# AcherStyx/SSD-Object-Detection

Measured on AMD Instinct MI355X. Metric: images/sec SSD300 train step, batch 64, higher is better.
Workload: dtype bf16; 1 GPU; BASELINE configs[2]: SSD300 full train step (anchor match+encode, image normalisation, conv fwd, loss, conv bwd, per-variable clip (64 variables) + Adam), per-GPU batch 64, 80 classes, synthetic COCO-shaped boxes; per_gpu_batch=64, global_batch=64, parallelism=single

## Files before the change

include/ssd_hip.h:

```cpp
#ifndef SSD_HIP_H
#define SSD_HIP_H

#include <stddef.h>
#include <stdint.h>

#ifdef __cplusplus
extern "C" {
#endif

typedef enum {
    SSD_OK = 0,
    SSD_ERR_ASSERT = -1,
    SSD_ERR_VALUE = -2,
    SSD_ERR_WORKSPACE = -3,
    SSD_ERR_LAUNCH = -4,
    SSD_ERR_UNSUPPORTED = -5
} ssd_status;

typedef enum { SSD_F32 = 0, SSD_BF16 = 1 } ssd_dtype;

int ssd_hip_abi_version(void);
const char* ssd_status_string(int status);

int ssd_priors_count(const int* grid_hw, int levels, const int* ratio_off);
// ... 88 lines not shown
    const void* x;
    const void* dy;
    float* dw;
    float* dbias;
    int B, H, W, Cin, Cout, ldy, ksize, stride, pad_t, pad_l, Ho, Wo;
} ssd_wgrad_item;
size_t ssd_conv2d_bwd_weight_batched_workspace_bytes(const ssd_wgrad_item* items, int count);
int ssd_conv2d_bwd_weight_batched(const ssd_wgrad_item* items, int count, void* ws, size_t ws_bytes, void* stream);
int ssd_set_wgrad_reduce_stream(void* stream);
int ssd_weight_transpose(const void* w, void* w_t, int Cout, int ksize, int Cin, int Cout_pad, void* stream);
int ssd_weight_transpose_batched(const long long* desc, int ntensors, int max_tiles, void* stream);
int ssd_cast_bf16(const float* src, void* dst, long long n, void* stream);
int ssd_image_prep(const float* img, void* out, int B, int H, int W, int normalize, void* stream);
int ssd_image_resize_prep(const void* src, const int64_t* src_off, const int32_t* src_hw, void* out, int B, int S,
                          int normalize, void* stream);
int ssd_box_prep(const float* box_tlwh, const int32_t* gt_off, const int32_t* src_hw, float* box_out, int B, int total_gt,
                 void* stream);
int ssd_maxpool2x2_fwd(const void* x, void* y, int B, int H, int W, int C, int Ho, int Wo, void* stream);
int ssd_maxpool2x2_bwd(const void* x, const void* y, const void* dy, void* dx, int B, int H, int W, int C, int Ho,
                       int Wo, void* stream);
int ssd_maxpool2x2_fwd_argmax(const void* x, void* y, void* code, int B, int H, int W, int C, int Ho, int Wo, void* stream);
int ssd_maxpool2x2_bwd_argmax(const void* code, const void* dy, void* dx, int B, int H, int W, int C, int Ho, int Wo,
                              void* stream);
int ssd_quantize_mx_fp8(const void* x_bf16, void* q, void* scale, long long n, void* stream);
int ssd_conv3x3_fwd_mxfp8(const void* x8, const void* xscale, const void* w8, const void* wscale, const float* bias, void* y, int B,
                          int H, int W, int Cin, int Cout, int relu, void* stream);
#define SSD_CHAIN_MAX_LAYERS 8
#define SSD_CHAIN_PACK_MAX 16
typedef struct {
    const void* src;
    void* dst;
    int N, K;
} ssd_chain_pack;
int ssd_chain_pack_weights(const ssd_chain_pack* items, int count, void* stream);
int ssd_chain_prefetch(const ssd_chain_pack* items, int count, void* stream);
typedef struct {
    const void* w;
    const float* bias;
    void* out;
    const void* mask_bits;
    const void* mask_src;
    void* relu_bits;
    int Hi, Wi, Kc, Ho, Wo, N, ksize, mul, div, pad_t, pad_l, relu, accumulate;
} ssd_chain_layer;
int ssd_conv_chain(const void* in0, const ssd_chain_layer* layers, int nlayers, int B, void* stream);
int ssd_add_relu_fwd(const void* a, const void* b, void* out, long long n, void* stream);
int ssd_relu_mask_bwd(const void* g, const void* act, void* out, int accumulate, long long n, void* stream);
int ssd_maxpool3x3s2_fwd(const void* x, void* y, void* code, int B, int H, int W, int C, int Ho, int Wo, int pad_t, int pad_l,
                         void* stream);
int ssd_maxpool3x3s2_bwd(const void* code, const void* dy, void* dx, int B, int H, int W, int C, int Ho, int Wo, int pad_t, int pad_l,
                         void* stream);
typedef struct {
    int levels;
    int H[SSD_MAX_LEVELS], W[SSD_MAX_LEVELS], Cin[SSD_MAX_LEVELS], cout[SSD_MAX_LEVELS];
    const void* x[SSD_MAX_LEVELS];
    const void* w_tap[SSD_MAX_LEVELS];
    const void* relu_bits[SSD_MAX_LEVELS];
    const void* relu_src[SSD_MAX_LEVELS];
    void* dx[SSD_MAX_LEVELS];
    float* dw[SSD_MAX_LEVELS];
    float* dbias[SSD_MAX_LEVELS];
} ssd_head_layers;
size_t ssd_heads_bwd_data_sparse_workspace_bytes(int B, const ssd_head_layers* hl);
int ssd_heads_bwd_data_sparse(const ssd_head_grads* hg, const ssd_head_layers* hl, int B, void* ws, size_t ws_bytes,
                              void* stream);
int ssd_heads_bwd_data_sparse_levels(const ssd_head_grads* hg, const ssd_head_layers* hl, int B, unsigned level_mask, int prezeroed,
                                     void* ws, size_t ws_bytes, void* stream);
size_t ssd_heads_bwd_weight_sparse_workspace_bytes(int B, const ssd_head_grads* hg, const ssd_head_layers* hl);
int ssd_heads_bwd_weight_sparse(const ssd_head_grads* hg, const ssd_head_layers* hl, int B, void* ws, size_t ws_bytes,
                                void* stream);

int ssd_head_grad_pack(const void* dloc, const void* dconf, void* out, int B, int hw, int per_cell, int classes,
                       int npad, int anchors_total, int level_off, void* stream);

int ssd_opt_block_elems(void);
int ssd_grad_clip_scales(const float* grad, long long n, const int32_t* tensor_block_off, int ntensors, float clip,
                         double* partial, float* scale, float* norms, void* stream);
int ssd_grad_apply_scale(float* grad, long long n, const int32_t* block_tensor, const float* scale, void* stream);
int ssd_grad_accumulate(float* acc, const float* grad, long long n, const int32_t* block_tensor, const float* scale,
                        int first, void* stream);
int ssd_adam_step(float* param, const float* grad, float* m, float* v, void* param_bf16, long long n,
                  const int32_t* block_tensor, const float* scale, float grad_scale, float lr_t, float beta1,
                  float beta2, float eps, void* stream);
int ssd_sgd_step(float* param, const float* grad, void* param_bf16, long long n, const int32_t* block_tensor,
                 const float* scale, float grad_scale, float lr, void* stream);

enum ssd_conv_plan {
    SSD_PLAN_KERNEL_MASK = 0xff,
    SSD_PLAN_C64B = 1, SSD_PLAN_P32_64, SSD_PLAN_P32_128, SSD_PLAN_8PH,
    SSD_PLAN_DMA_256_256, SSD_PLAN_DMA_256_128, SSD_PLAN_DMA_256_64, SSD_PLAN_DMA_128_64, SSD_PLAN_DMA_128_128,
    SSD_PLAN_CONV0_FWD, SSD_PLAN_P512, SSD_PLAN_PW,
    SSD_PLAN_WG_FIRST = 32, SSD_PLAN_WG_PATCH_16x16, SSD_PLAN_WG_PATCH_6x40, SSD_PLAN_WG_PATCH_10x24, SSD_PLAN_WG_TILE,
    SSD_PLAN_WG_GENERIC,
    SSD_PLAN_F_FLAT = 0x100,
    SSD_PLAN_F_ROWFLAT = 0x200,
    SSD_PLAN_F_SPLITK = 0x400,
    SSD_PLAN_F_POOL_FUSED = 0x800,
    SSD_PLAN_F_S2 = 0x1000,
    SSD_PLAN_F_REDUCE_WIDE = 0x2000
};
int ssd_conv2d_fwd_plan(int B, int H, int W, int Cin, int Cout, int ksize, int stride, int pad_t, int pad_l, int Ho, int Wo,
                        int pool, size_t ws_bytes);
int ssd_conv2d_head_fwd_plan(int B, int H, int W, int Cin, int per_cell, int classes, size_t ws_bytes);
int ssd_conv2d_bwd_data_plan(int B, int H, int W, int Cin, int Cout_pad, int ksize, int stride, int pad_t, int pad_l, int Ho,
                             int Wo, int accumulate, size_t ws_bytes);
int ssd_conv2d_bwd_weight_plan(int B, int H, int W, int Cin, int Cout, int ldy, int ksize, int stride, int pad_t, int pad_l,
                               int Ho, int Wo);
const char* ssd_conv_plan_name(int plan);

int ssd_dev_knob(const char* name, int value);

int ssd_dev_mfma_calibration_workgroups(void);
double ssd_dev_mfma_calibration_flops(int iters);
int ssd_dev_mfma_calibration(int iters, void* stamps, void* sink, void* stream);

#ifdef __cplusplus
}
#endif
#endif
```

ssd-object-detection_amd/_lib.py:

```python
import ctypes
import os

HERE = os.path.dirname(os.path.abspath(__file__))
LIB_PATH = os.path.join(HERE, os.environ.get("SSD_HIP_LIB", "libssd_hip.so"))

SSD_OK, SSD_ERR_ASSERT, SSD_ERR_VALUE, SSD_ERR_WORKSPACE, SSD_ERR_LAUNCH, SSD_ERR_UNSUPPORTED = 0, -1, -2, -3, -4, -5
SSD_MAX_LEVELS = 8

_c_int_p = ctypes.POINTER(ctypes.c_int)
_c_double_p = ctypes.POINTER(ctypes.c_double)
VP = ctypes.c_void_p


class PriorGrid(ctypes.Structure):
    _fields_ = [("levels", ctypes.c_int),
                ("grid_h", ctypes.c_int * SSD_MAX_LEVELS),
                ("grid_w", ctypes.c_int * SSD_MAX_LEVELS),
                ("per_cell", ctypes.c_int * SSD_MAX_LEVELS),
                ("verified", ctypes.c_int)]


class HeadGrads(ctypes.Structure):
    _fields_ = [("levels", ctypes.c_int),
                ("hw", ctypes.c_int * SSD_MAX_LEVELS),
# ... 17 lines not shown
                ("relu_src", VP * SSD_MAX_LEVELS),
                ("dx", VP * SSD_MAX_LEVELS),
                ("dw", VP * SSD_MAX_LEVELS),
                ("dbias", VP * SSD_MAX_LEVELS)]


class ChainLayer(ctypes.Structure):
    _fields_ = [("w", VP), ("bias", VP), ("out", VP), ("mask_bits", VP), ("mask_src", VP), ("relu_bits", VP)] + \
               [(n, ctypes.c_int) for n in ("Hi", "Wi", "Kc", "Ho", "Wo", "N", "ksize", "mul", "div", "pad_t", "pad_l", "relu",
                                            "accumulate")]


class WgradItem(ctypes.Structure):
    _fields_ = [("x", VP), ("dy", VP), ("dw", VP), ("dbias", VP)] + \
               [(n, ctypes.c_int) for n in ("B", "H", "W", "Cin", "Cout", "ldy", "ksize", "stride", "pad_t", "pad_l", "Ho", "Wo")]


class ChainPack(ctypes.Structure):
    _fields_ = [("src", VP), ("dst", VP), ("N", ctypes.c_int), ("K", ctypes.c_int)]


SSD_CHAIN_MAX_LAYERS = 8
SSD_CHAIN_PACK_MAX = 16
_HG = ctypes.POINTER(HeadGrads)
_HL = ctypes.POINTER(HeadLayers)

_SIGNATURES = {
    "ssd_hip_abi_version": (ctypes.c_int, []),
    "ssd_status_string": (ctypes.c_char_p, [ctypes.c_int]),
    "ssd_priors_count": (ctypes.c_int, [_c_int_p, ctypes.c_int, _c_int_p]),
    "ssd_priors": (ctypes.c_int, [_c_int_p, ctypes.c_int, _c_double_p, _c_int_p, _c_int_p, ctypes.c_double, VP, VP]),
    "ssd_encode_zero": (ctypes.c_int, [VP, ctypes.c_int, VP, VP]),
    "ssd_prior_grid_verify": (ctypes.c_int, [VP, ctypes.c_int, ctypes.POINTER(PriorGrid), VP, VP]),
    "ssd_match_encode_workspace_bytes": (ctypes.c_size_t, [ctypes.c_int, ctypes.c_int, ctypes.c_int]),
    "ssd_match_encode": (ctypes.c_int, [VP, VP, VP, ctypes.c_int, ctypes.c_int, ctypes.c_int, VP, VP, ctypes.c_int,
                                        ctypes.POINTER(PriorGrid), ctypes.c_double, VP, VP, VP, VP, VP, ctypes.c_size_t, VP]),
    "ssd_apply_anchor_box": (ctypes.c_int, [VP, VP, ctypes.c_int, VP, VP]),
    "ssd_iou_n": (ctypes.c_int, [VP, VP, ctypes.c_int, VP, VP]),
    "ssd_score_decode": (ctypes.c_int, [VP, VP, ctypes.c_int, VP, ctypes.c_int, ctypes.c_int, ctypes.c_int,
                                        ctypes.c_float, ctypes.c_double, VP, VP, VP, VP, VP]),
    "ssd_nms_max_candidates": (ctypes.c_int, []),
    "ssd_nms": (ctypes.c_int, [VP, VP, VP, VP, ctypes.c_int, ctypes.c_int, ctypes.c_float, ctypes.c_int, VP, VP, VP]),
    "ssd_conv2d_fwd": (ctypes.c_int, [VP, VP, VP, VP] + [ctypes.c_int] * 12 + [VP, ctypes.c_size_t, VP]),
    "ssd_conv2d_fwd_pool": (ctypes.c_int, [VP, VP, VP, VP, VP, VP] + [ctypes.c_int] * 14 + [VP, ctypes.c_size_t, VP]),
    "ssd_conv2d_head_fwd": (ctypes.c_int, [VP, VP, VP, VP, VP] + [ctypes.c_int] * 8 + [VP, ctypes.c_size_t, VP]),
    "ssd_conv2d_bwd_data": (ctypes.c_int, [VP, VP, VP, VP] + [ctypes.c_int] * 12 + [VP, ctypes.c_size_t, VP]),
    "ssd_conv2d_fwd_relubits": (ctypes.c_int, [VP] * 5 + [ctypes.c_int] * 11 + [VP, ctypes.c_size_t, VP]),
    "ssd_conv2d_bwd_data_bits": (ctypes.c_int, [VP] * 4 + [ctypes.c_int] * 12 + [VP, ctypes.c_size_t, VP]),
    "ssd_conv2d_bwd_data_unpool": (ctypes.c_int, [VP] * 6 + [ctypes.c_int] * 7 + [VP, ctypes.c_size_t, VP]),
    "ssd_quantize_mx_fp8": (ctypes.c_int, [VP, VP, VP, ctypes.c_longlong, VP]),
    "ssd_conv3x3_fwd_mxfp8": (ctypes.c_int, [VP] * 6 + [ctypes.c_int] * 6 + [VP]),
    "ssd_chain_pack_weights": (ctypes.c_int, [ctypes.POINTER(ChainPack), ctypes.c_int, VP]),
    "ssd_chain_prefetch": (ctypes.c_int, [ctypes.POINTER(ChainPack), ctypes.c_int, VP]),
    "ssd_set_wgrad_reduce_stream": (ctypes.c_int, [VP]),
    "ssd_conv2d_bwd_weight_batched_workspace_bytes": (ctypes.c_size_t, [ctypes.POINTER(WgradItem), ctypes.c_int]),
    "ssd_conv2d_bwd_weight_batched": (ctypes.c_int, [ctypes.POINTER(WgradItem), ctypes.c_int, VP, ctypes.c_size_t, VP]),
    "ssd_conv_chain": (ctypes.c_int, [VP, ctypes.POINTER(ChainLayer), ctypes.c_int, ctypes.c_int, VP]),
    "ssd_add_relu_fwd": (ctypes.c_int, [VP, VP, VP, ctypes.c_longlong, VP]),
    "ssd_relu_mask_bwd": (ctypes.c_int, [VP, VP, VP, ctypes.c_int, ctypes.c_longlong, VP]),
    "ssd_maxpool3x3s2_fwd": (ctypes.c_int, [VP, VP, VP] + [ctypes.c_int] * 8 + [VP]),
    "ssd_maxpool3x3s2_bwd": (ctypes.c_int, [VP, VP, VP] + [ctypes.c_int] * 8 + [VP]),
    "ssd_conv2d_bwd_weight_unpooled_workspace_bytes": (ctypes.c_size_t, [ctypes.c_int] * 7),
    "ssd_conv2d_bwd_weight_unpooled": (ctypes.c_int, [VP] * 5 + [ctypes.c_int] * 7 + [VP, ctypes.c_size_t, VP]),
    "ssd_conv2d_bwd_data_wgrad_first_workspace_bytes": (ctypes.c_size_t, [ctypes.c_int] * 3),
    "ssd_conv2d_bwd_data_wgrad_first": (ctypes.c_int, [VP] * 6 + [ctypes.c_int] * 3 + [VP, ctypes.c_size_t, VP]),
    "ssd_conv2d_bwd_weight_workspace_bytes": (ctypes.c_size_t, [ctypes.c_int] * 7),
    "ssd_conv2d_bwd_weight": (ctypes.c_int, [VP, VP, VP, VP] + [ctypes.c_int] * 12 + [VP, ctypes.c_size_t, VP]),
    "ssd_weight_transpose": (ctypes.c_int, [VP, VP, ctypes.c_int, ctypes.c_int, ctypes.c_int, ctypes.c_int, VP]),
    "ssd_cast_bf16": (ctypes.c_int, [VP, VP, ctypes.c_longlong, VP]),
    "ssd_image_prep": (ctypes.c_int, [VP, VP, ctypes.c_int, ctypes.c_int, ctypes.c_int, ctypes.c_int, VP]),
    "ssd_image_resize_prep": (ctypes.c_int, [VP, VP, VP, VP, ctypes.c_int, ctypes.c_int, ctypes.c_int, VP]),
    "ssd_box_prep": (ctypes.c_int, [VP, VP, VP, VP, ctypes.c_int, ctypes.c_int, VP]),
    "ssd_maxpool2x2_fwd": (ctypes.c_int, [VP, VP] + [ctypes.c_int] * 6 + [VP]),
    "ssd_maxpool2x2_bwd": (ctypes.c_int, [VP, VP, VP, VP] + [ctypes.c_int] * 6 + [VP]),
    "ssd_weight_transpose_batched": (ctypes.c_int, [VP, ctypes.c_int, ctypes.c_int, VP]),
    "ssd_maxpool2x2_fwd_argmax": (ctypes.c_int, [VP, VP, VP] + [ctypes.c_int] * 6 + [VP]),
    "ssd_maxpool2x2_bwd_argmax": (ctypes.c_int, [VP, VP, VP] + [ctypes.c_int] * 6 + [VP]),
    "ssd_head_grad_pack": (ctypes.c_int, [VP, VP, VP] + [ctypes.c_int] * 7 + [VP]),
    "ssd_opt_block_elems": (ctypes.c_int, []),
    "ssd_grad_clip_scales": (ctypes.c_int, [VP, ctypes.c_longlong, VP, ctypes.c_int, ctypes.c_float, VP, VP, VP, VP]),
    "ssd_grad_apply_scale": (ctypes.c_int, [VP, ctypes.c_longlong, VP, VP, VP]),
    "ssd_grad_accumulate": (ctypes.c_int, [VP, VP, ctypes.c_longlong, VP, VP, ctypes.c_int, VP]),
    "ssd_adam_step": (ctypes.c_int, [VP, VP, VP, VP, VP, ctypes.c_longlong, VP, VP] + [ctypes.c_float] * 5 + [VP]),
    "ssd_sgd_step": (ctypes.c_int, [VP, VP, VP, ctypes.c_longlong, VP, VP, ctypes.c_float, ctypes.c_float, VP]),
    "ssd_dev_knob": (ctypes.c_int, [ctypes.c_char_p, ctypes.c_int]),
    "ssd_dev_mfma_calibration_workgroups": (ctypes.c_int, []),
    "ssd_dev_mfma_calibration_flops": (ctypes.c_double, [ctypes.c_int]),
    "ssd_dev_mfma_calibration": (ctypes.c_int, [ctypes.c_int, VP, VP, VP]),
    "ssd_conv2d_fwd_plan": (ctypes.c_int, [ctypes.c_int] * 12 + [ctypes.c_size_t]),
    "ssd_conv2d_head_fwd_plan": (ctypes.c_int, [ctypes.c_int] * 6 + [ctypes.c_size_t]),
    "ssd_conv2d_bwd_data_plan": (ctypes.c_int, [ctypes.c_int] * 12 + [ctypes.c_size_t]),
    "ssd_conv2d_bwd_weight_plan": (ctypes.c_int, [ctypes.c_int] * 12),
    "ssd_conv_plan_name": (ctypes.c_char_p, [ctypes.c_int]),
    "ssd_loss_workspace_bytes": (ctypes.c_size_t, [ctypes.c_int, ctypes.c_int, ctypes.c_int]),
    "ssd_loss_heads_workspace_bytes": (ctypes.c_size_t, [ctypes.c_int, ctypes.c_int, ctypes.c_int]),
    "ssd_loss_fwd_bwd_heads": (ctypes.c_int, [VP, VP, ctypes.c_int, VP, VP, VP, ctypes.c_int, ctypes.c_int, ctypes.c_int,
                                              ctypes.c_float, VP, _HG, VP, ctypes.c_size_t, ctypes.c_int, VP]),
    "ssd_heads_bwd_data_sparse_workspace_bytes": (ctypes.c_size_t, [ctypes.c_int, _HL]),
    "ssd_heads_bwd_data_sparse": (ctypes.c_int, [_HG, _HL, ctypes.c_int, VP, ctypes.c_size_t, VP]),
    "ssd_heads_bwd_data_sparse_levels": (ctypes.c_int, [_HG, _HL, ctypes.c_int, ctypes.c_uint, ctypes.c_int, VP, ctypes.c_size_t, VP]),
    "ssd_heads_bwd_weight_sparse_workspace_bytes": (ctypes.c_size_t, [ctypes.c_int, _HG, _HL]),
    "ssd_heads_bwd_weight_sparse": (ctypes.c_int, [_HG, _HL, ctypes.c_int, VP, ctypes.c_size_t, VP]),
    "ssd_loss_fwd_bwd": (ctypes.c_int, [VP, VP, ctypes.c_int, VP, VP, VP, ctypes.c_int, ctypes.c_int, ctypes.c_int,
                                        ctypes.c_float, VP, VP, VP, VP, ctypes.c_size_t, VP]),
}

_lib = None


def lib():
    global _lib
    if _lib is None:
        if not os.path.exists(LIB_PATH):
            raise RuntimeError(
                "libssd_hip.so is missing (%s): build it with `python ssd-object-detection_amd/build.py` "
                "or __graft_entry__.build(); there is no CPU fallback." % LIB_PATH)
        try:
            import torch
        except ImportError:
            pass
        L = ctypes.CDLL(LIB_PATH)
        for name, (res, args) in _SIGNATURES.items():
            fn = getattr(L, name)
            fn.restype = res
            fn.argtypes = args
        _lib = L
    return _lib


def check(status):
    if status == SSD_OK:
        return
    msg = lib().ssd_status_string(status).decode()
    if status == SSD_ERR_ASSERT:
        raise AssertionError(msg)
    if status in (SSD_ERR_VALUE, SSD_ERR_UNSUPPORTED):
        raise ValueError(msg)
    raise RuntimeError("ssd_hip: %s (status %d)" % (msg, status))
```

ssd-object-detection_amd/csrc/optim.hip:

```cpp
#include "common.h"
#include <hip/hip_bf16.h>

namespace {

constexpr int OPT_BLOCK = 1024;

__device__ __forceinline__ unsigned short f2bf_bits(float f) {
    const __hip_bfloat16 h = __float2bfloat16(f);
    return *reinterpret_cast<const unsigned short*>(&h);
}

__global__ __launch_bounds__(256) void k_sqnorm_partial(const float* __restrict__ g, long long n, double* __restrict__ partial) {
    __shared__ double s_red[4];
    const long long i = ((long long)blockIdx.x * 256 + threadIdx.x) * 4;
    double s = 0.0;
    if (i + 3 < n) {
        const float4 v = *reinterpret_cast<const float4*>(g + i);
        s = (double)v.x * v.x + (double)v.y * v.y + (double)v.z * v.z + (double)v.w * v.w;
    } else {
        for (long long k = i; k < n; ++k) s += (double)g[k] * g[k];
    }
#pragma unroll
    for (int off = 32; off > 0; off >>= 1) {
        const int lo = __shfl_xor(__double2loint(s), off);
        const int hi = __shfl_xor(__double2hiint(s), off);
        s += __hiloint2double(hi, lo);
    }
    if ((threadIdx.x & 63) == 0) s_red[threadIdx.x >> 6] = s;
    __syncthreads();
    if (threadIdx.x == 0) partial[blockIdx.x] = s_red[0] + s_red[1] + s_red[2] + s_red[3];
}

__global__ __launch_bounds__(256) void k_clip_scale(const double* __restrict__ partial, const int* __restrict__ tensor_block_off,
                                                    int ntensors, float clip, float* __restrict__ scale,
                                                    float* __restrict__ norms) {
    __shared__ double s_red[256];
    const int t = blockIdx.x;
    if (t >= ntensors) return;
    const int b0 = tensor_block_off[t], b1 = tensor_block_off[t + 1];
    double s = 0.0;
    for (int b = b0 + threadIdx.x; b < b1; b += 256) s += partial[b];
    s_red[threadIdx.x] = s;
    __syncthreads();
    for (int off = 128; off > 0; off >>= 1) {
        if (threadIdx.x < off) s_red[threadIdx.x] += s_red[threadIdx.x + off];
        __syncthreads();
    }
    if (threadIdx.x == 0) {
        const float nrm = (float)sqrt(s_red[0]);
        if (norms) norms[t] = nrm;
        scale[t] = clip > 0.f ? clip / fmaxf(nrm, clip) : 1.f;
    }
}

__global__ __launch_bounds__(256) void k_apply_scale(float* __restrict__ g, long long n, const int* __restrict__ block_tensor,
                                                     const float* __restrict__ scale) {
    const long long i = ((long long)blockIdx.x * 256 + threadIdx.x) * 4;
    if (i >= n) return;
    const float sc = scale[block_tensor[blockIdx.x]];
    float4 v = *reinterpret_cast<float4*>(g + i);
    v.x *= sc; v.y *= sc; v.z *= sc; v.w *= sc;
    *reinterpret_cast<float4*>(g + i) = v;
}

__global__ __launch_bounds__(256) void k_accumulate(float* __restrict__ acc, const float* __restrict__ g, long long n,
                                                    const int* __restrict__ block_tensor, const float* __restrict__ scale,
                                                    int first) {
    const long long i = ((long long)blockIdx.x * 256 + threadIdx.x) * 4;
    if (i >= n) return;
    const float sc = scale ? scale[block_tensor[blockIdx.x]] : 1.f;
    const float4 gv = *reinterpret_cast<const float4*>(g + i);
    float4 a = first ? make_float4(0.f, 0.f, 0.f, 0.f) : *reinterpret_cast<float4*>(acc + i);
    a.x += gv.x * sc; a.y += gv.y * sc; a.z += gv.z * sc; a.w += gv.w * sc;
    *reinterpret_cast<float4*>(acc + i) = a;
}

__global__ __launch_bounds__(256) void k_adam(float* __restrict__ p, const float* __restrict__ g, float* __restrict__ m,
                                              float* __restrict__ v, unsigned short* __restrict__ p_bf16, long long n,
                                              const int* __restrict__ block_tensor, const float* __restrict__ scale,
                                              float grad_scale, float lr_t, float b1, float b2, float eps) {
    const long long i = ((long long)blockIdx.x * 256 + threadIdx.x) * 4;
    if (i >= n) return;
    const float sc = grad_scale * (scale ? scale[block_tensor[blockIdx.x]] : 1.f);
    const float4 gv = *reinterpret_cast<const float4*>(g + i);
    float4 pv = *reinterpret_cast<float4*>(p + i);
    float4 mv = *reinterpret_cast<float4*>(m + i);
    float4 vv = *reinterpret_cast<float4*>(v + i);
    const float gs[4] = {gv.x * sc, gv.y * sc, gv.z * sc, gv.w * sc};
    float* pp = reinterpret_cast<float*>(&pv);
    float* mm = reinterpret_cast<float*>(&mv);
    float* vq = reinterpret_cast<float*>(&vv);
#pragma unroll
    for (int k = 0; k < 4; ++k) {
        mm[k] = b1 * mm[k] + (1.f - b1) * gs[k];
        vq[k] = b2 * vq[k] + (1.f - b2) * gs[k] * gs[k];
        pp[k] -= lr_t * mm[k] / (sqrtf(vq[k]) + eps);
    }
    *reinterpret_cast<float4*>(p + i) = pv;
    *reinterpret_cast<float4*>(m + i) = mv;
    *reinterpret_cast<float4*>(v + i) = vv;
    if (p_bf16)
        *reinterpret_cast<uint2*>(p_bf16 + i) = make_uint2((unsigned)f2bf_bits(pp[0]) | ((unsigned)f2bf_bits(pp[1]) << 16),
                                                           (unsigned)f2bf_bits(pp[2]) | ((unsigned)f2bf_bits(pp[3]) << 16));
}

__global__ __launch_bounds__(256) void k_sgd(float* __restrict__ p, const float* __restrict__ g, unsigned short* __restrict__ p_bf16,
                                             long long n, const int* __restrict__ block_tensor, const float* __restrict__ scale,
                                             float grad_scale, float lr) {
    const long long i = ((long long)blockIdx.x * 256 + threadIdx.x) * 4;
    if (i >= n) return;
    const float sc = grad_scale * (scale ? scale[block_tensor[blockIdx.x]] : 1.f);
    const float4 gv = *reinterpret_cast<const float4*>(g + i);
    float4 pv = *reinterpret_cast<float4*>(p + i);
    pv.x -= lr * gv.x * sc; pv.y -= lr * gv.y * sc; pv.z -= lr * gv.z * sc; pv.w -= lr * gv.w * sc;
    *reinterpret_cast<float4*>(p + i) = pv;
    if (p_bf16)
        *reinterpret_cast<uint2*>(p_bf16 + i) = make_uint2((unsigned)f2bf_bits(pv.x) | ((unsigned)f2bf_bits(pv.y) << 16),
                                                           (unsigned)f2bf_bits(pv.z) | ((unsigned)f2bf_bits(pv.w) << 16));
}

}

extern "C" {

int ssd_opt_block_elems(void) { return OPT_BLOCK; }

int ssd_grad_clip_scales(const float* grad, long long n, const int32_t* tensor_block_off, int ntensors, float clip,
                         double* partial, float* scale, float* norms, void* stream) {
    if (!grad || !tensor_block_off || !partial || !scale || n <= 0 || n % OPT_BLOCK || ntensors <= 0) return SSD_ERR_VALUE;
    const unsigned nb = (unsigned)(n / OPT_BLOCK);
    hipStream_t s = (hipStream_t)stream;
    hipLaunchKernelGGL(k_sqnorm_partial, dim3(nb), dim3(256), 0, s, grad, n, partial);
    hipLaunchKernelGGL(k_clip_scale, dim3(ntensors), dim3(256), 0, s, partial, tensor_block_off, ntensors, clip,
                       scale, norms);
    return ssd_launch_status();
}

int ssd_grad_apply_scale(float* grad, long long n, const int32_t* block_tensor, const float* scale, void* stream) {
    if (!grad || !block_tensor || !scale || n <= 0 || n % OPT_BLOCK) return SSD_ERR_VALUE;
    hipLaunchKernelGGL(k_apply_scale, dim3((unsigned)(n / OPT_BLOCK)), dim3(256), 0, (hipStream_t)stream, grad, n,
                       block_tensor, scale);
    return ssd_launch_status();
}

int ssd_grad_accumulate(float* acc, const float* grad, long long n, const int32_t* block_tensor, const float* scale,
                        int first, void* stream) {
    if (!acc || !grad || n <= 0 || n % OPT_BLOCK || (scale && !block_tensor)) return SSD_ERR_VALUE;
    hipLaunchKernelGGL(k_accumulate, dim3((unsigned)(n / OPT_BLOCK)), dim3(256), 0, (hipStream_t)stream, acc, grad, n,
                       block_tensor, scale, first);
    return ssd_launch_status();
}

int ssd_adam_step(float* param, const float* grad, float* m, float* v, void* param_bf16, long long n,
                  const int32_t* block_tensor, const float* scale, float grad_scale, float lr_t, float beta1, float beta2,
                  float eps, void* stream) {
    if (!param || !grad || !m || !v || n <= 0 || n % OPT_BLOCK || (scale && !block_tensor)) return SSD_ERR_VALUE;
    hipLaunchKernelGGL(k_adam, dim3((unsigned)(n / OPT_BLOCK)), dim3(256), 0, (hipStream_t)stream, param, grad, m, v,
                       static_cast<unsigned short*>(param_bf16), n, block_tensor, scale, grad_scale, lr_t, beta1, beta2, eps);
    return ssd_launch_status();
}

int ssd_sgd_step(float* param, const float* grad, void* param_bf16, long long n, const int32_t* block_tensor,
                 const float* scale, float grad_scale, float lr, void* stream) {
    if (!param || !grad || n <= 0 || n % OPT_BLOCK || (scale && !block_tensor)) return SSD_ERR_VALUE;
    hipLaunchKernelGGL(k_sgd, dim3((unsigned)(n / OPT_BLOCK)), dim3(256), 0, (hipStream_t)stream, param, grad,
                       static_cast<unsigned short*>(param_bf16), n, block_tensor, scale, grad_scale, lr);
    return ssd_launch_status();
}

}
```

ssd-object-detection_amd/engine.py:

```python
import ctypes
import math
import os

import numpy as np
import torch

from . import _lib, ops

SSD300_TRUNK = [
    ("conv", 8, 64, 3, 1, "same", False),
    ("conv", 64, 64, 3, 1, "same", False),
    ("pool", 64, 64, 2, 2, "valid", False),
    ("conv", 64, 128, 3, 1, "same", False),
    ("conv", 128, 128, 3, 1, "same", False),
    ("pool", 128, 128, 2, 2, "valid", False),
    ("conv", 128, 256, 3, 1, "same", False),
    ("conv", 256, 256, 3, 1, "same", False),
    ("conv", 256, 256, 3, 1, "same", False),
    ("pool", 256, 256, 2, 2, "same", False),
    ("conv", 256, 512, 3, 1, "same", False),
    ("conv", 512, 512, 3, 1, "same", False),
    ("conv", 512, 512, 1, 1, "same", True),
    ("conv", 512, 1024, 3, 2, "same", False),
    ("conv", 1024, 1024, 1, 1, "same", True),
# ... 138 lines not shown
        for i, nd in enumerate(self.nodes):
            if nd["kind"] != "conv":
                continue
            self.conv_params[i] = (add("conv%d/kernel" % i, (nd["cout"], nd["k"], nd["k"], nd["cin"])),
                                   add("conv%d/bias" % i, (nd["cout"],)))
        self.head_params = []
        for lvl, ((_, h, c), n) in enumerate(zip(self.fm, self.num_priors)):
            nl, nc = n * 4, n * self.classes
            lk, ck = add("head%d/loc_kernel" % lvl, (nl, 3, 3, c), True), add("head%d/conf_kernel" % lvl, (nc, 3, 3, c))
            lb, cb = add("head%d/loc_bias" % lvl, (nl,), True), add("head%d/conf_bias" % lvl, (nc,))
            self.head_params.append((FusedView("head%d/kernel" % lvl, (nl + nc, 3, 3, c), (lk, ck)),
                                     FusedView("head%d/bias" % lvl, (nl + nc,), (lb, cb))))
        self.n_flat = off
        self.n_params = sum(t.numel for t in self.tensors)

    def _alloc_params(self):
        dev, n = self.device, self.n_flat
        self.param = torch.zeros(n, dtype=torch.float32, device=dev)
        self.grad = torch.zeros(n, dtype=torch.float32, device=dev)
        self.grad_acc = None
        self.adam_m = torch.zeros(n, dtype=torch.float32, device=dev)
        self.adam_v = torch.zeros(n, dtype=torch.float32, device=dev)
        self.param_bf16 = torch.zeros(n, dtype=torch.bfloat16, device=dev)
        nb = n // self.block
        tbo = np.zeros(len(self.tensors) + 1, np.int32)
        bt = np.zeros(nb, np.int32)
        for i, t in enumerate(self.tensors):
            b0, b1 = t.block0, t.block0 + t.nblocks
            tbo[i], tbo[i + 1] = b0, b1
            bt[b0:b1] = i
        self.tensor_block_off = torch.from_numpy(tbo).to(dev)
        self.block_tensor = torch.from_numpy(bt).to(dev)
        self.sq_partial = torch.empty(nb, dtype=torch.float64, device=dev)
        self.clip_scale = torch.empty(len(self.tensors), dtype=torch.float32, device=dev)
        self.grad_norms = torch.empty(len(self.tensors), dtype=torch.float32, device=dev)
        self.w_t = {}
        for i, nd in enumerate(self.nodes):
            if nd["kind"] == "conv" and i > 0:
                self.w_t[i] = torch.empty((nd["cin"], nd["k"], nd["k"], nd["cout"]), dtype=torch.bfloat16, device=dev)
        self.chain_pk_fwd, self.chain_pk_bwd = {}, {}
        if getattr(self, "chain_start", None) is not None and self.chain:
            for i in range(self.chain_start, len(self.nodes)):
                nd = self.nodes[i]
                self.chain_pk_fwd[i] = torch.empty((nd["cout"], nd["k"], nd["k"], nd["cin"]), dtype=torch.bfloat16, device=dev)
                self.chain_pk_bwd[i] = torch.empty_like(self.w_t[i])
        self.head_npad = [(n * (4 + self.classes) + 7) // 8 * 8 for n in self.num_priors]
        self.head_w_t = [torch.empty((3, 3, c, npad) if self.sparse_heads else (c, 3, 3, npad), dtype=torch.bfloat16, device=dev)
                         for (_, _, c), npad in zip(self.fm, self.head_npad)]

    def view(self, t, buf):
        return buf[t.offset:t.offset + t.numel].view(t.shape)

    def init_params(self, seed=0):
        rng = np.random.default_rng(seed)
        host = np.zeros(self.n_flat, np.float32)
        for t in self.tensors:
            if not t.name.endswith("kernel"):
                continue
            cout, k, _, cin = t.shape
            if t.name.startswith("head"):
                lim = math.sqrt(6.0 / (k * k * cin + k * k * cout))
                w = rng.uniform(-lim, lim, (cout, k, k, cin))
            else:
                real_cin = IMAGE_CHANNELS if t.name == "conv0/kernel" else cin
                lim = math.sqrt(6.0 / (k * k * real_cin + k * k * cout))
                w = rng.uniform(-lim, lim, (cout, k, k, cin))
                if real_cin != cin:
                    w[..., real_cin:] = 0.0
            host[t.offset:t.offset + t.numel] = w.astype(np.float32).reshape(-1)
        self.param.copy_(torch.from_numpy(host))
        self.adam_m.zero_()
        self.adam_v.zero_()
        self.step_count = 0
        self.refresh_weights(cast=True)

    def refresh_weights(self, cast=False, tensors=None):
        if cast:
            ops.cast_bf16(self.param, self.param_bf16)
        if getattr(self, "_tr_desc", None) is None:
            rows, tiles = [], 0
            pairs = [(self.conv_params[i][0], wt) for i, wt in self.w_t.items()]
            n_trunk = len(pairs)
            pairs += [(self.head_params[lvl][0], wt) for lvl, wt in enumerate(self.head_w_t)]
            for r, (pt, wt) in enumerate(pairs):
                cout, k, _, cin = pt.shape
                cpad = wt.shape[-1]
                kfield = k | (0x100 if (self.sparse_heads and r >= n_trunk) else 0)
                rows.append([self.view(pt, self.param_bf16).data_ptr(), wt.data_ptr(), cout, kfield, cin, cpad])
                tiles = max(tiles, ((cpad + 31) // 32) * ((cin + 31) // 32) * k * k)
            self._tr_desc = torch.tensor(rows, dtype=torch.int64, device=self.device)
            self._tr_tiles = tiles
            self._tr_tensor = [pt.index for pt, _ in pairs]
        r0, r1 = 0, self._tr_desc.shape[0]
        if tensors is not None:
            inside = [r for r, t in enumerate(self._tr_tensor) if tensors[0] <= t < tensors[1]]
            if not inside:
                return
            r0, r1 = inside[0], inside[-1] + 1
            assert inside == list(range(r0, r1))
        _lib.check(self.L.ssd_weight_transpose_batched(ops._ptr(self._tr_desc[r0:]), r1 - r0, self._tr_tiles,
                                                       ops._stream()))
        if self.chain_pk_fwd:
            items = []
            for i in self.chain_pk_fwd:
                wt = self.conv_params[i][0]
                if tensors is None or tensors[0] <= wt.index < tensors[1]:
                    items += [(self.view(wt, self.param_bf16), self.chain_pk_fwd[i]), (self.w_t[i], self.chain_pk_bwd[i])]
            if items:
                ops.chain_pack_weights(items)

    def _acts(self, B):
        c = self._act_cache.get(B)
        if c is None:
            dev = self.device
            acts = [None]
            gacts = [None]
            for nd in self.nodes:
                shape = (B, nd["hout"], nd["hout"], nd["cout"])
                acts.append(torch.empty(shape, dtype=torch.bfloat16, device=dev))
                gacts.append(torch.empty(shape, dtype=torch.bfloat16, device=dev))
            loc = torch.empty((B, self.A, 4), dtype=torch.bfloat16, device=dev)
            conf = torch.empty((B, self.A, self.classes), dtype=torch.bfloat16, device=dev)
            packed = [torch.empty((B, h * h, npad), dtype=torch.bfloat16, device=dev)
                      for (_, h, _), npad in zip(self.fm, self.head_npad)]
            pool_code = {i: torch.empty((B, nd["hout"], nd["hout"], nd["cout"] // 8), dtype=torch.int32, device=dev)
                         for i, nd in enumerate(self.nodes) if nd["kind"] == "pool"}
            rbits = {i + 1: torch.empty((B, nd["hout"], nd["hout"], nd["cout"] // 8), dtype=torch.uint8, device=dev)
                     for i, nd in enumerate(self.nodes) if nd["kind"] == "conv" and nd["cout"] % 8 == 0}
            hgb = None
            if self.sparse_heads:
                hgb = ops.HeadGradBuffers(B, [h * h for _, h, _ in self.fm], self.num_priors, self.head_npad, device=dev)
            c = dict(acts=acts, gacts=gacts, loc=loc, conf=conf, packed=packed, pool_code=pool_code, rbits=rbits, hgb=hgb)
            self._act_cache = {B: c}
        return c

    SIDE_HEADS = (0, 1)

    def _side_stream(self):
        if getattr(self, "_side", None) is None:
            self._side = torch.cuda.Stream(device=self.device, priority=int(os.environ.get("SSD_SIDE_PRIO", "0")))
            self._ws_side = ops.MatchWorkspace()
        return self._side

    def forward(self, x):
        B = x.shape[0]
        c = self._acts(B)
        acts = c["acts"]
        acts[0] = x
        main = torch.cuda.current_stream()
        side = self._side_stream() if self.overlap_heads else None
        tail = None
        if side is not None and self.tail_stream:
            if getattr(self, "_tail", None) is None:
                self._tail = torch.cuda.Stream(device=self.device)
                self._ws_tail = ops.MatchWorkspace()
            tail = self._tail
        fm_level = {ni: lvl for lvl, (ni, _, _) in enumerate(self.fm)}

        def head(lvl, ws):
            ni = self.fm[lvl][0]
            wt, bt = self.head_params[lvl]
            ops.conv2d_head_fwd(acts[ni + 1], self.view(wt, self.param_bf16), self.view(bt, self.param), c["loc"],
                                c["conf"], self.num_priors[lvl], self.classes, self.level_off[lvl], ws=ws)

        def after_node(i):
            lvl = fm_level.get(i)
            if side is not None and lvl in self.SIDE_HEADS:
                ev = torch.cuda.Event()
                ev.record(main)
                with torch.cuda.stream(side):
                    side.wait_event(ev)
                    head(lvl, self._ws_side)
            elif tail is not None and lvl is not None:
                ev = torch.cuda.Event()
                ev.record(main)
                with torch.cuda.stream(tail):
                    tail.wait_event(ev)
                    head(lvl, self._ws_tail)

        self.bits_valid = set()
        self._prezeroed = set()
        big_maps = [ni + 1 for lvl, (ni, h, ch) in enumerate(self.fm) if B * h * h >= 16384]
        clear_at = min(9, len(self.nodes) - 1)
        for i, nd in enumerate(self.nodes):
# ... 460 lines not shown
                    continue
                except NotImplementedError:
                    self.fuse_first = False
            prev_is_relu_conv = self.nodes[i - 1]["kind"] == "conv"
            if i in head_done:
                main.wait_event(head_done.pop(i))
            if i in sparse_head_done:
                main.wait_event(sparse_head_done.pop(i))
            fused = False
            if (self.fuse_unpool is not None and self.fuse_unpool.get(i, True) and self.nodes[i - 1]["kind"] == "pool" and not written[i] and not written[i - 1]
                    and nd["k"] == 3 and nd["stride"] == 1 and nd["pt"] == 1 and nd["pl"] == 1):
                try:
                    ops.conv2d_bwd_data_unpool(g_out, self.w_t[i], None, c["pool_code"][i - 1], tuple(gacts[i - 1].shape),
                                               out=gacts[i - 1], ws=self._ws)
                    fused = True
                    unpooled.add(i - 1)
                except NotImplementedError:
                    pass
                self.fuse_unpool[i] = fused
            if not fused and prev_is_relu_conv:
                masked_dgrad("conv%d" % i, g_out, self.w_t[i], i, nd["stride"], nd["pt"], nd["pl"], written[i], self._ws)
            elif not fused:
                ops.conv2d_bwd_data(g_out, self.w_t[i], None, acts[i].shape, nd["stride"], nd["pt"], nd["pl"],
                                    accumulate=written[i], out=gacts[i], ws=self._ws)
            written[i] = True
            opt_bucket(i)
        assert not opt_at
        flush_side()
        if prefetch_done is not None:
            main.wait_event(prefetch_done)
        for ev in sparse_head_done.values():
            main.wait_event(ev)
        for t0, t1, ev, ev2 in deferred:
            main.wait_event(ev)
            if ev2 is not None:
                main.wait_event(ev2)
            self.adam_range(t0, t1, lr_t, hp["beta1"], hp["beta2"], hp["eps"], hp["clip"])
        if side is not None:
            main.wait_stream(side)
            if side2 is not None:
                main.wait_stream(side2)
            if red is not None:
                main.wait_stream(red)
                _lib.check(self.L.ssd_set_wgrad_reduce_stream(None))
                self._red_active = None

    def clip_scales(self, clip=0.01):
        _lib.check(self.L.ssd_grad_clip_scales(ops._ptr(self.grad), self.n_flat, ops._ptr(self.tensor_block_off),
                                               len(self.tensors), float(clip), ops._ptr(self.sq_partial),
                                               ops._ptr(self.clip_scale), ops._ptr(self.grad_norms), ops._stream()))

    def apply_clip_in_place(self):
        _lib.check(self.L.ssd_grad_apply_scale(ops._ptr(self.grad), self.n_flat, ops._ptr(self.block_tensor),
                                               ops._ptr(self.clip_scale), ops._stream()))

    def _range_table(self, t0, t1):
        key = (t0, t1)
        if not hasattr(self, "_range_tables"):
            self._range_tables = {}
        tab = self._range_tables.get(key)
        if tab is None:
            b0 = self.tensors[t0].block0
            tbo = (self.tensor_block_off[t0:t1 + 1] - b0).contiguous()
            bt = (self.block_tensor[b0:int(self.tensor_block_off[t1].item())] - t0).contiguous()
            tab = (b0, tbo, bt)
            self._range_tables[key] = tab
        return tab

    def opt_buckets(self, min_elems=2_000_000):
        if getattr(self, "_opt_buckets", None) is None:
            first_head = self.head_params[0][0].index
            out = [(first_head, len(self.tensors), None)]
            hi, acc = first_head, 0
            conv_nodes = sorted(self.conv_params)
            for i in reversed(conv_nodes):
                wt, bt = self.conv_params[i]
                acc += wt.numel + bt.numel
                if acc >= min_elems or i == conv_nodes[0]:
                    out.append((wt.index, hi, i))
                    hi, acc = wt.index, 0
            self._opt_buckets = out
        return self._opt_buckets

    def adam_range(self, t0, t1, lr_t, beta1, beta2, eps, clip, grad_scale=1.0):
        b0, tbo, bt = self._range_table(t0, t1)
        start, n = b0 * self.block, bt.numel() * self.block
        sl = slice(start, start + n)
        if clip is not None:
            _lib.check(self.L.ssd_grad_clip_scales(ops._ptr(self.grad[sl]), n, ops._ptr(tbo), t1 - t0, float(clip),
                                                   ops._ptr(self.sq_partial[b0:]), ops._ptr(self.clip_scale[t0:]),
                                                   ops._ptr(self.grad_norms[t0:]), ops._stream()))
        _lib.check(self.L.ssd_adam_step(ops._ptr(self.param[sl]), ops._ptr(self.grad[sl]), ops._ptr(self.adam_m[sl]),
                                        ops._ptr(self.adam_v[sl]), ops._ptr(self.param_bf16[sl]), n, ops._ptr(bt),
                                        ops._ptr(self.clip_scale[t0:]) if clip is not None else None, float(grad_scale),
                                        float(lr_t), float(beta1), float(beta2), float(eps), ops._stream()))
        self.refresh_weights(tensors=(t0, t1))

    def clip_range_in_place(self, t0, t1, clip=0.01):
        b0, tbo, bt = self._range_table(t0, t1)
        start = b0 * self.block
        n = bt.numel() * self.block
        g = self.grad[start:start + n]
        _lib.check(self.L.ssd_grad_clip_scales(ops._ptr(g), n, ops._ptr(tbo), t1 - t0, float(clip),
                                               ops._ptr(self.sq_partial[b0:]), ops._ptr(self.clip_scale[t0:]),
                                               ops._ptr(self.grad_norms[t0:]), ops._stream()))
        _lib.check(self.L.ssd_grad_apply_scale(ops._ptr(g), n, ops._ptr(bt), ops._ptr(self.clip_scale[t0:]), ops._stream()))

    def accumulate_clipped(self, first):
        if self.grad_acc is None:
            self.grad_acc = torch.empty_like(self.grad)
        _lib.check(self.L.ssd_grad_accumulate(ops._ptr(self.grad_acc), ops._ptr(self.grad), self.n_flat,
                                              ops._ptr(self.block_tensor), ops._ptr(self.clip_scale), 1 if first else 0,
                                              ops._stream()))

    def adam(self, lr, grad, grad_scale=1.0, use_clip_scale=False, beta1=0.9, beta2=0.999, eps=1e-7):
        self.step_count += 1
        t = self.step_count
        lr_t = lr * math.sqrt(1.0 - beta2 ** t) / (1.0 - beta1 ** t)
        _lib.check(self.L.ssd_adam_step(ops._ptr(self.param), ops._ptr(grad), ops._ptr(self.adam_m), ops._ptr(self.adam_v),
                                        ops._ptr(self.param_bf16), self.n_flat, ops._ptr(self.block_tensor),
                                        ops._ptr(self.clip_scale) if use_clip_scale else None, float(grad_scale),
                                        float(lr_t), float(beta1), float(beta2), float(eps), ops._stream()))
        self.refresh_weights()

    def sgd(self, lr, grad, grad_scale=1.0, use_clip_scale=False):
        self.step_count += 1
        _lib.check(self.L.ssd_sgd_step(ops._ptr(self.param), ops._ptr(grad), ops._ptr(self.param_bf16), self.n_flat,
                                       ops._ptr(self.block_tensor), ops._ptr(self.clip_scale) if use_clip_scale else None,
                                       float(grad_scale), float(lr), ops._stream()))
        self.refresh_weights()

    LAYOUT_VERSION = 2

    def state_dict(self):
        return dict(param=self.param.cpu(), adam_m=self.adam_m.cpu(), adam_v=self.adam_v.cpu(), step=self.step_count,
                    names=[t.name for t in self.tensors], shapes=[t.shape for t in self.tensors],
                    offsets=[t.offset for t in self.tensors], layout_version=self.LAYOUT_VERSION)

    def load_state_dict(self, sd):
        mine = ([t.name for t in self.tensors], [tuple(t.shape) for t in self.tensors], [t.offset for t in self.tensors])
        theirs = (list(sd.get("names", [])), [tuple(x) for x in sd.get("shapes", [])], list(sd.get("offsets", [])))
        if sd.get("layout_version", 1) != self.LAYOUT_VERSION or mine != theirs or sd["param"].numel() != self.n_flat:
            bad = [n for n in mine[0] if n not in theirs[0]][:3] + [n for n in theirs[0] if n not in mine[0]][:3]
            raise ValueError("checkpoint parameter layout (version %s, %d variables, %d elements) does not match this engine's "
                             "(version %d, %d variables, %d elements)%s" % (
                                 sd.get("layout_version", 1), len(theirs[0]), sd["param"].numel(), self.LAYOUT_VERSION,
                                 len(mine[0]), self.n_flat, "; e.g. " + ", ".join(bad) if bad else ""))
        self.param.copy_(sd["param"])
        self.adam_m.copy_(sd["adam_m"])
        self.adam_v.copy_(sd["adam_v"])
        self.step_count = int(sd["step"])
        self.refresh_weights(cast=True)
```

Before: 7112 images/sec.

## Fuse Adam update with bf16 cast and weight transpose into one finalize kernel

Adds a segmented finalize kernel that runs the Adam update on tiles of each conv weight, writes the bf16 copy, and writes the transposed backward-weight layout through a shared-memory tile in the same launch. A host-built segment table covers the non-weight remainder (biases and other tensors) with plain vectorised Adam blocks. This replaces the separate Adam-then-batched-transpose sequence and removes one pass that re-reads the bf16 weights. The cost is a more complex indexing scheme, a fallback path when a tensor group is split across ranges, and per-tile scale selection for fused parameter parts.

```diff
diff --git a/include/ssd_hip.h b/include/ssd_hip.h
--- a/include/ssd_hip.h
+++ b/include/ssd_hip.h
@@ -194,6 +194,9 @@
 int ssd_adam_step(float* param, const float* grad, float* m, float* v, void* param_bf16, long long n,
                   const int32_t* block_tensor, const float* scale, float grad_scale, float lr_t, float beta1,
                   float beta2, float eps, void* stream);
+int ssd_adam_finalize(const long long* seg, const int32_t* item_seg, int nitems, float* param, const float* grad, float* m,
+                      float* v, void* param_bf16, const float* scale, float grad_scale, float lr_t, float beta1, float beta2,
+                      float eps, void* stream);
 int ssd_sgd_step(float* param, const float* grad, void* param_bf16, long long n, const int32_t* block_tensor,
                  const float* scale, float grad_scale, float lr, void* stream);
 
diff --git a/ssd-object-detection_amd/_lib.py b/ssd-object-detection_amd/_lib.py
--- a/ssd-object-detection_amd/_lib.py
+++ b/ssd-object-detection_amd/_lib.py
@@ -123,6 +123,7 @@
     "ssd_grad_apply_scale": (ctypes.c_int, [VP, ctypes.c_longlong, VP, VP, VP]),
     "ssd_grad_accumulate": (ctypes.c_int, [VP, VP, ctypes.c_longlong, VP, VP, ctypes.c_int, VP]),
     "ssd_adam_step": (ctypes.c_int, [VP, VP, VP, VP, VP, ctypes.c_longlong, VP, VP] + [ctypes.c_float] * 5 + [VP]),
+    "ssd_adam_finalize": (ctypes.c_int, [VP, VP, ctypes.c_int, VP, VP, VP, VP, VP, VP] + [ctypes.c_float] * 5 + [VP]),
     "ssd_sgd_step": (ctypes.c_int, [VP, VP, VP, ctypes.c_longlong, VP, VP, ctypes.c_float, ctypes.c_float, VP]),
     "ssd_dev_knob": (ctypes.c_int, [ctypes.c_char_p, ctypes.c_int]),
     "ssd_dev_mfma_calibration_workgroups": (ctypes.c_int, []),
diff --git a/ssd-object-detection_amd/csrc/optim.hip b/ssd-object-detection_amd/csrc/optim.hip
--- a/ssd-object-detection_amd/csrc/optim.hip
+++ b/ssd-object-detection_amd/csrc/optim.hip
@@ -10,8 +10,7 @@
     return *reinterpret_cast<const unsigned short*>(&h);
 }
 
-__global__ __launch_bounds__(256) void k_sqnorm_partial(const float* __restrict__ g, long long n, double* __restrict__ partial) {
-    __shared__ double s_red[4];
+__device__ __forceinline__ double block_sqnorm(const float* __restrict__ g, long long n, double* s_red) {
     const long long i = ((long long)blockIdx.x * 256 + threadIdx.x) * 4;
     double s = 0.0;
     if (i + 3 < n) {
@@ -28,16 +27,11 @@
     }
     if ((threadIdx.x & 63) == 0) s_red[threadIdx.x >> 6] = s;
     __syncthreads();
-    if (threadIdx.x == 0) partial[blockIdx.x] = s_red[0] + s_red[1] + s_red[2] + s_red[3];
-}
-
-__global__ __launch_bounds__(256) void k_clip_scale(const double* __restrict__ partial, const int* __restrict__ tensor_block_off,
-                                                    int ntensors, float clip, float* __restrict__ scale,
-                                                    float* __restrict__ norms) {
-    __shared__ double s_red[256];
-    const int t = blockIdx.x;
-    if (t >= ntensors) return;
-    const int b0 = tensor_block_off[t], b1 = tensor_block_off[t + 1];
+    return s_red[0] + s_red[1] + s_red[2] + s_red[3];
+}
+
+__device__ __forceinline__ void tensor_clip_scale(const double* partial, int b0, int b1, float clip, float* __restrict__ scale,
+                                                  float* __restrict__ norm, double* s_red) {
     double s = 0.0;
     for (int b = b0 + threadIdx.x; b < b1; b += 256) s += partial[b];
     s_red[threadIdx.x] = s;
@@ -48,9 +42,24 @@
     }
     if (threadIdx.x == 0) {
         const float nrm = (float)sqrt(s_red[0]);
-        if (norms) norms[t] = nrm;
-        scale[t] = clip > 0.f ? clip / fmaxf(nrm, clip) : 1.f;
-    }
+        if (norm) *norm = nrm;
+        *scale = clip > 0.f ? clip / fmaxf(nrm, clip) : 1.f;
+    }
+}
+
+__global__ __launch_bounds__(256) void k_sqnorm_partial(const float* __restrict__ g, long long n, double* __restrict__ partial) {
+    __shared__ double s_red[4];
+    const double s = block_sqnorm(g, n, s_red);
+    if (threadIdx.x == 0) partial[blockIdx.x] = s;
+}
+
+__global__ __launch_bounds__(256) void k_clip_scale(const double* __restrict__ partial, const int* __restrict__ tensor_block_off,
+                                                    int ntensors, float clip, float* __restrict__ scale,
+                                                    float* __restrict__ norms) {
+    __shared__ double s_red[256];
+    const int t = blockIdx.x;
+    if (t >= ntensors) return;
+    tensor_clip_scale(partial, tensor_block_off[t], tensor_block_off[t + 1], clip, scale + t, norms ? norms + t : nullptr, s_red);
 }
 
 __global__ __launch_bounds__(256) void k_apply_scale(float* __restrict__ g, long long n, const int* __restrict__ block_tensor,
@@ -73,6 +82,12 @@
     float4 a = first ? make_float4(0.f, 0.f, 0.f, 0.f) : *reinterpret_cast<float4*>(acc + i);
     a.x += gv.x * sc; a.y += gv.y * sc; a.z += gv.z * sc; a.w += gv.w * sc;
     *reinterpret_cast<float4*>(acc + i) = a;
+}
+
+__device__ __forceinline__ void adam_elem(float& p, float& m, float& v, float g, float lr_t, float b1, float b2, float eps) {
+    m = b1 * m + (1.f - b1) * g;
+    v = b2 * v + (1.f - b2) * g * g;
+    p -= lr_t * m / (sqrtf(v) + eps);
 }
 
 __global__ __launch_bounds__(256) void k_adam(float* __restrict__ p, const float* __restrict__ g, float* __restrict__ m,
@@ -91,17 +106,91 @@
     float* mm = reinterpret_cast<float*>(&mv);
     float* vq = reinterpret_cast<float*>(&vv);
 #pragma unroll
-    for (int k = 0; k < 4; ++k) {
-        mm[k] = b1 * mm[k] + (1.f - b1) * gs[k];
-        vq[k] = b2 * vq[k] + (1.f - b2) * gs[k] * gs[k];
-        pp[k] -= lr_t * mm[k] / (sqrtf(vq[k]) + eps);
-    }
+    for (int k = 0; k < 4; ++k) adam_elem(pp[k], mm[k], vq[k], gs[k], lr_t, b1, b2, eps);
     *reinterpret_cast<float4*>(p + i) = pv;
     *reinterpret_cast<float4*>(m + i) = mv;
     *reinterpret_cast<float4*>(v + i) = vv;
     if (p_bf16)
         *reinterpret_cast<uint2*>(p_bf16 + i) = make_uint2((unsigned)f2bf_bits(pp[0]) | ((unsigned)f2bf_bits(pp[1]) << 16),
                                                            (unsigned)f2bf_bits(pp[2]) | ((unsigned)f2bf_bits(pp[3]) << 16));
+}
+
+constexpr int FIN_ROW = 12;
+
+__device__ __forceinline__ void adam4(float* __restrict__ p, const float* __restrict__ g, float* __restrict__ m,
+                                      float* __restrict__ v, long long i, float sc, float lr_t, float b1, float b2, float eps,
+                                      float4& out) {
+    const float4 gv = *reinterpret_cast<const float4*>(g + i);
+    float4 pv = *reinterpret_cast<float4*>(p + i);
+    float4 mv = *reinterpret_cast<float4*>(m + i);
+    float4 vv = *reinterpret_cast<float4*>(v + i);
+    const float gs[4] = {gv.x * sc, gv.y * sc, gv.z * sc, gv.w * sc};
+    float* pp = reinterpret_cast<float*>(&pv);
+    float* mm = reinterpret_cast<float*>(&mv);
+    float* vq = reinterpret_cast<float*>(&vv);
+#pragma unroll
+    for (int k = 0; k < 4; ++k) adam_elem(pp[k], mm[k], vq[k], gs[k], lr_t, b1, b2, eps);
+    *reinterpret_cast<float4*>(p + i) = pv;
+    *reinterpret_cast<float4*>(m + i) = mv;
+    *reinterpret_cast<float4*>(v + i) = vv;
+    out = pv;
+}
+
+__global__ __launch_bounds__(256) void k_adam_finalize(const long long* __restrict__ seg, const int* __restrict__ item_seg,
+                                                       float* __restrict__ p, const float* __restrict__ g, float* __restrict__ m,
+                                                       float* __restrict__ v, unsigned short* __restrict__ p_bf16,
+                                                       const float* __restrict__ scale, float grad_scale, float lr_t, float b1,
+                                                       float b2, float eps) {
+    __shared__ unsigned short tile[32][33];
+    const long long* d = seg + (long long)item_seg[blockIdx.x] * FIN_ROW;
+    const int kind = (int)d[0];
+    const long long e0 = d[1];
+    const int local = (int)(blockIdx.x - d[11]);
+    if (kind == 0) {
+        const long long i = e0 + (long long)local * 1024 + threadIdx.x * 4;
+        if (i >= e0 + d[2]) return;
+        const float sc = grad_scale * (scale ? scale[(int)d[3]] : 1.f);
+        float4 pv;
+        adam4(p, g, m, v, i, sc, lr_t, b1, b2, eps, pv);
+        *reinterpret_cast<uint2*>(p_bf16 + i) = make_uint2((unsigned)f2bf_bits(pv.x) | ((unsigned)f2bf_bits(pv.y) << 16),
+                                                           (unsigned)f2bf_bits(pv.z) | ((unsigned)f2bf_bits(pv.w) << 16));
+        return;
+    }
+    unsigned short* wt = reinterpret_cast<unsigned short*>(d[6]);
+    const int Cout = (int)d[7], K = (int)d[8] & 0xff, tapmajor = ((int)d[8] >> 8) & 1, Cin = (int)d[9], Cout_pad = (int)d[10];
+    const int tci = (Cin + 31) >> 5;
+    int t = local;
+    const int tap = t % (K * K); t /= K * K;
+    const int ci0 = (t % tci) * 32, co0 = (t / tci) * 32;
+    const int kh = tap / K, kw = tap - kh * K;
+    {
+        const int r = threadIdx.x >> 3, c = (threadIdx.x & 7) * 4;
+        const int co = co0 + r, ci = ci0 + c;
+        uint2 bf = make_uint2(0u, 0u);
+        if (co < Cout && ci < Cin) {
+            const float sc = grad_scale * (scale ? scale[co < (int)d[5] ? (int)d[3] : (int)d[4]] : 1.f);
+            const long long i = e0 + (((long long)co * K + kh) * K + kw) * Cin + ci;
+            float4 pv;
+            adam4(p, g, m, v, i, sc, lr_t, b1, b2, eps, pv);
+            bf = make_uint2((unsigned)f2bf_bits(pv.x) | ((unsigned)f2bf_bits(pv.y) << 16),
+                            (unsigned)f2bf_bits(pv.z) | ((unsigned)f2bf_bits(pv.w) << 16));
+            *reinterpret_cast<uint2*>(p_bf16 + i) = bf;
+        }
+        tile[r][c] = (unsigned short)(bf.x & 0xffff);
+        tile[r][c + 1] = (unsigned short)(bf.x >> 16);
+        tile[r][c + 2] = (unsigned short)(bf.y & 0xffff);
+        tile[r][c + 3] = (unsigned short)(bf.y >> 16);
+    }
+    __syncthreads();
+    const int dkh = tapmajor ? kh : K - 1 - kh, dkw = tapmajor ? kw : K - 1 - kw;
+    const int tx = threadIdx.x & 31, ty = threadIdx.x >> 5;
+#pragma unroll
+    for (int j = 0; j < 4; ++j) {
+        const int ci = ci0 + ty + 8 * j, co = co0 + tx;
+        if (ci >= Cin || co >= Cout_pad) continue;
+        if (tapmajor) wt[(((long long)dkh * K + dkw) * Cin + ci) * Cout_pad + co] = tile[tx][ty + 8 * j];
+        else wt[(((long long)ci * K + dkh) * K + dkw) * Cout_pad + co] = tile[tx][ty + 8 * j];
+    }
 }
 
 __global__ __launch_bounds__(256) void k_sgd(float* __restrict__ p, const float* __restrict__ g, unsigned short* __restrict__ p_bf16,
@@ -160,6 +249,15 @@
     return ssd_launch_status();
 }
 
+int ssd_adam_finalize(const long long* seg, const int32_t* item_seg, int nitems, float* param, const float* grad, float* m,
+                      float* v, void* param_bf16, const float* scale, float grad_scale, float lr_t, float beta1, float beta2,
+                      float eps, void* stream) {
+    if (!seg || !item_seg || nitems <= 0 || !param || !grad || !m || !v || !param_bf16) return SSD_ERR_VALUE;
+    hipLaunchKernelGGL(k_adam_finalize, dim3((unsigned)nitems), dim3(256), 0, (hipStream_t)stream, seg, item_seg, param, grad,
+                       m, v, static_cast<unsigned short*>(param_bf16), scale, grad_scale, lr_t, beta1, beta2, eps);
+    return ssd_launch_status();
+}
+
 int ssd_sgd_step(float* param, const float* grad, void* param_bf16, long long n, const int32_t* block_tensor,
                  const float* scale, float grad_scale, float lr, void* stream) {
     if (!param || !grad || n <= 0 || n % OPT_BLOCK || (scale && !block_tensor)) return SSD_ERR_VALUE;
diff --git a/ssd-object-detection_amd/engine.py b/ssd-object-detection_amd/engine.py
--- a/ssd-object-detection_amd/engine.py
+++ b/ssd-object-detection_amd/engine.py
@@ -244,12 +244,14 @@
             pairs = [(self.conv_params[i][0], wt) for i, wt in self.w_t.items()]
             n_trunk = len(pairs)
             pairs += [(self.head_params[lvl][0], wt) for lvl, wt in enumerate(self.head_w_t)]
+            self._tr_pairs = []
             for r, (pt, wt) in enumerate(pairs):
                 cout, k, _, cin = pt.shape
                 cpad = wt.shape[-1]
                 kfield = k | (0x100 if (self.sparse_heads and r >= n_trunk) else 0)
                 rows.append([self.view(pt, self.param_bf16).data_ptr(), wt.data_ptr(), cout, kfield, cin, cpad])
                 tiles = max(tiles, ((cpad + 31) // 32) * ((cin + 31) // 32) * k * k)
+                self._tr_pairs.append((pt, wt, kfield))
             self._tr_desc = torch.tensor(rows, dtype=torch.int64, device=self.device)
             self._tr_tiles = tiles
             self._tr_tensor = [pt.index for pt, _ in pairs]
@@ -262,6 +264,9 @@
             assert inside == list(range(r0, r1))
         _lib.check(self.L.ssd_weight_transpose_batched(ops._ptr(self._tr_desc[r0:]), r1 - r0, self._tr_tiles,
                                                        ops._stream()))
+        self._chain_pack(tensors)
+
+    def _chain_pack(self, tensors=None):
         if self.chain_pk_fwd:
             items = []
             for i in self.chain_pk_fwd:
@@ -888,6 +893,50 @@
             self._opt_buckets = out
         return self._opt_buckets
 
+    def _finalize_table(self, t0, t1):
+        key = (t0, t1)
+        if not hasattr(self, "_fin_tables"):
+            self._fin_tables = {}
+        if key in self._fin_tables:
+            return self._fin_tables[key]
+        if getattr(self, "_tr_desc", None) is None:
+            self.refresh_weights()
+        base = self.tensors[t0].block0 * self.block
+        rows, item_seg, covered = [], [], {}
+
+        def add(nitems, row):
+            item_seg.extend([len(rows)] * nitems)
+            rows.append(row + [len(item_seg) - nitems])
+
+        for pt, wt, kfield in self._tr_pairs:
+            parts = getattr(pt, "parts", (pt,))
+            inside = [t0 <= q.index < t1 for q in parts]
+            if not any(inside):
+                continue
+            if not all(inside):
+                self._fin_tables[key] = None
+                return None
+            cout, k, _, cin = pt.shape
+            cpad = wt.shape[-1]
+            assert cin % 4 == 0 and pt.offset % 4 == 0
+            tiles = ((cpad + 31) // 32) * ((cin + 31) // 32) * k * k
+            add(tiles, [1, pt.offset - base, pt.numel, parts[0].index - t0, parts[-1].index - t0, parts[0].shape[0],
+                        wt.data_ptr(), cout, kfield, cin, cpad])
+            for q in parts:
+                covered[q.index] = (q.offset, q.offset + q.numel)
+        for t in range(t0, t1):
+            T = self.tensors[t]
+            lo, hi = T.block0 * self.block, (T.block0 + T.nblocks) * self.block
+            c0, c1 = covered.get(t, (hi, hi))
+            for a, b in ((lo, c0), (c1, hi)):
+                if b > a:
+                    assert a % 4 == 0 and (b - a) % 4 == 0
+                    add((b - a + self.block - 1) // self.block, [0, a - base, b - a, t - t0, t - t0, 0, 0, 0, 0, 0, 0])
+        tab = (torch.tensor(rows, dtype=torch.int64, device=self.device),
+               torch.tensor(item_seg, dtype=torch.int32, device=self.device), len(item_seg))
+        self._fin_tables[key] = tab
+        return tab
+
     def adam_range(self, t0, t1, lr_t, beta1, beta2, eps, clip, grad_scale=1.0):
         b0, tbo, bt = self._range_table(t0, t1)
         start, n = b0 * self.block, bt.numel() * self.block
@@ -896,11 +945,21 @@
             _lib.check(self.L.ssd_grad_clip_scales(ops._ptr(self.grad[sl]), n, ops._ptr(tbo), t1 - t0, float(clip),
                                                    ops._ptr(self.sq_partial[b0:]), ops._ptr(self.clip_scale[t0:]),
                                                    ops._ptr(self.grad_norms[t0:]), ops._stream()))
-        _lib.check(self.L.ssd_adam_step(ops._ptr(self.param[sl]), ops._ptr(self.grad[sl]), ops._ptr(self.adam_m[sl]),
-                                        ops._ptr(self.adam_v[sl]), ops._ptr(self.param_bf16[sl]), n, ops._ptr(bt),
-                                        ops._ptr(self.clip_scale[t0:]) if clip is not None else None, float(grad_scale),
-                                        float(lr_t), float(beta1), float(beta2), float(eps), ops._stream()))
-        self.refresh_weights(tensors=(t0, t1))
+        fin = self._finalize_table(t0, t1)
+        if fin is None:
+            _lib.check(self.L.ssd_adam_step(ops._ptr(self.param[sl]), ops._ptr(self.grad[sl]), ops._ptr(self.adam_m[sl]),
+                                            ops._ptr(self.adam_v[sl]), ops._ptr(self.param_bf16[sl]), n, ops._ptr(bt),
+                                            ops._ptr(self.clip_scale[t0:]) if clip is not None else None, float(grad_scale),
+                                            float(lr_t), float(beta1), float(beta2), float(eps), ops._stream()))
+            self.refresh_weights(tensors=(t0, t1))
+            return
+        seg, item_seg, nitems = fin
+        _lib.check(self.L.ssd_adam_finalize(ops._ptr(seg), ops._ptr(item_seg), nitems, ops._ptr(self.param[sl]),
+                                            ops._ptr(self.grad[sl]), ops._ptr(self.adam_m[sl]), ops._ptr(self.adam_v[sl]),
+                                            ops._ptr(self.param_bf16[sl]),
+                                            ops._ptr(self.clip_scale[t0:]) if clip is not None else None, float(grad_scale),
+                                            float(lr_t), float(beta1), float(beta2), float(eps), ops._stream()))
+        self._chain_pack(tensors=(t0, t1))
 
     def clip_range_in_place(self, t0, t1, clip=0.01):
         b0, tbo, bt = self._range_table(t0, t1)
```

Result: no change. 7114 images/sec, median of 6 (+0.0%).
